# jonaselgammal/GPry

Measured on AMD Instinct MI355X. Metric: gp_refit_plus_nora_acq_cycle_throughput, higher is better.
Workload: dtype f64

## Files before the change

### gpry_amd/csrc/common.h

```cpp
#pragma once
#include <hip/hip_runtime.h>
#include <stdint.h>
#include <stdio.h>
#include <string.h>
#include <math.h>
#include <string>
#include <vector>
#include <map>

#include "../../include/gpry_hip.h"

#define GPRY_THETA_MAX (2 + GPRY_MAX_DIM)
#define GPRY_BPAR_ROW (2 + GPRY_MAX_DIM)
#define GPRY_BPAR_WHITE (1 + GPRY_MAX_DIM)
#define GPRY_TILE 128
#define GPRY_NB 64

typedef double v4d __attribute__((ext_vector_type(4)));

struct StageTimer {
    double total_ms = 0.0;
    int64_t count = 0;
    std::vector<std::pair<hipEvent_t, hipEvent_t>> pending;
};
// ... 65 lines not shown
    double* dalpha_ = nullptr;
    double* dvec = nullptr;
    int* dinfo = nullptr;
    double* dparams = nullptr;

    double* gate_sv = nullptr; double* gate_coef = nullptr; double* gate_trust = nullptr;
    int64_t gate_nsv = 0, gate_sv_cap = 0;
    double gate_gamma = 0.0, gate_intercept = 0.0;
    int gate_positive_finite = 1, gate_has_trust = 0, gates_on = 0;

    int64_t sw_M = 0, sw_cap = 0;
    double* dXc = nullptr;
    uint8_t* dmask = nullptr;
    double *dy_all = nullptr, *dsig_all = nullptr, *dacq_all = nullptr;
    struct CandSet {
        int64_t M = 0, cap = 0;
        double* dXc = nullptr; uint8_t* dmask = nullptr;
        double *dy = nullptr, *dsig = nullptr, *dacq = nullptr;
    } pr;
    double* dXcs = nullptr;
    int64_t xcs_cap = 0;
    double* dYcs = nullptr;
    int64_t ycs_cap = 0;
    double xcenter[GPRY_MAX_DIM] = {0};
    double xsum[GPRY_MAX_DIM] = {0};
    double xlo[GPRY_MAX_DIM] = {0}, xhi[GPRY_MAX_DIM] = {0};
    int opt_cross_mfma = 1;
    double alpha_l2 = -1.0;
    double alpha_l1 = 0.0;
    double noise_min = 0.0;
    int panel_form = 0;
    int opt_cross_hybrid = 1;
    double panel_est[4] = {0, 0, 0, 2.5e-7};
    double* dKst = nullptr;
    int64_t kst_cap = 0;
    double* dG = nullptr;
    int64_t g_cap = 0;
    double* dsplit = nullptr;
    int64_t split_cap = 0;
    int opt_predict_split = 1;
    int opt_gemm_dma = 1;
    double* dpart = nullptr;
    int64_t part_cap = 0;
    unsigned long long* dkeys = nullptr; int64_t keys_cap = 0;
    unsigned int* dhist = nullptr;
    unsigned int* dselp = nullptr;
// ... 26 lines not shown
    void* trtri_pipe = nullptr;
    int64_t opt_gemm_streamk = 5632;
    int64_t opt_topk_host = 16384;
    int opt_factor_pipeline = 1;
    int opt_factor_pipeline_min = 1280;
    void* chol_plan = nullptr;

    void* srv = nullptr;
    int opt_predict_serve = 1;
    int64_t opt_serve_idle_us = 2000;
    int opt_mcmc_mapped = 0;
    int64_t opt_chol_stacked = 2048;
    int opt_chol_stacked_dense = 0;
    int opt_sweep_overlap = 0;
    int opt_sweep_upload = 1;
    const double* up_X = nullptr;
    const double* up_y = nullptr;
    int up_gates = 0;
    int opt_kb_rank = 1;
    int opt_predict_gates = 0;
    int opt_sweep_prune = 0;
    int opt_sweep_mean_bound = 1;
    int opt_sweep_screen = 1;
    int sw_pruned = 0;
    struct PruneState {
        int have_mask = 0;
        int form = 0;
        FinishParams fp = {};
        int64_t n_eval = 0;
        int64_t rounds = 0, evaluated_total = 0, completed = 0, last_K = 0;
        int64_t n_gidx = 0;
        int tau_done = 0;
        double tau = 0.0;
        int64_t survivors = -1;
        int ybound = 0;
        int64_t live_blocks = 0, blocks = 0;
        int64_t cert_blocks = 0;
    } prune;
    struct ModelSnap {
        double *dV = nullptr, *dalpha_ = nullptr, *dXs = nullptr, *dX = nullptr;
        int64_t v_cap = 0, a_cap = 0, xs_cap = 0, x_cap = 0;
        int64_t N = 0, Np = 0;
        int d = 0, dpad = 0, kernel_id = 0;
        bool white = false;
        double theta[GPRY_THETA_MAX] = {0};
        gpry_affine tf;
// ... 159 lines not shown
void gemm_parts_plan_free(GemmPartsPlan* pl);
int gemm_dma_parts_launch(gpry_ctx* ctx, const GemmArgs& g, bool a_trans, bool b_trans, int epi, const GemmPartsPlan& pl,
                          int64_t slice_stride);
int gemm_f64_launch(gpry_ctx* ctx, const GemmArgs& g, bool a_trans, bool b_trans, int epi);
int gemm64_launch(gpry_ctx* ctx, const GemmArgs& g, bool a_trans, bool b_trans, int epi);
int gemm_split_scratch(gpry_ctx* ctx, int nsplit, int64_t slice, double** buf);
int launch_trtri_diag(gpry_ctx* ctx, const double* L, double* V, int64_t Np, hipStream_t st, bool zero_right = false);
int ensure_pred_xs(gpry_ctx* ctx);
int launch_point_full(gpry_ctx* ctx, const double* x, int want_kinv, double* kstar, double* G, double* u, double* part,
                      double* mean_part, double* ss_part, double* out);
int launch_trtri_diag128(gpry_ctx* ctx, const double* L, double* V, int64_t Np, hipStream_t st, bool clear_right);
int launch_trtri_diag_range(gpry_ctx* ctx, const double* L, double* V, int64_t Np, int blk0, int nblk, hipStream_t st);
bool gemm_dma_usable(const GemmArgs& g, int M, int N, int K);
int gemm_dma_launch_product(gpry_ctx* ctx, const GemmArgs& g, bool a_trans, bool b_trans, int epi, dim3 grid);
int sweep_gemm_dma_sp_launch(gpry_ctx* ctx, const GemmArgs& g);

int upload_params(gpry_ctx* ctx, const double* theta);
int launch_scale_train(gpry_ctx* ctx);
int launch_kernel_train(gpry_ctx* ctx, double* K, int add_noise, double* U = nullptr);
int launch_kernel_rows(gpry_ctx* ctx, int64_t row0, int k, int64_t ldk, double* Bk, double* Cb);
int launch_cross_build(gpry_ctx* ctx, const double* Xc, int64_t m0, int64_t mc,
                       int64_t ldk, double* Kst, double* mean_part, int raw_affine,
                       hipStream_t st = nullptr);
int launch_cross_prepare(gpry_ctx* ctx);
int launch_cross_build_mfma(gpry_ctx* ctx, const double* Xc, int64_t m0, int64_t mc, int64_t ldk, double* Kst, double* mean_part,
                            int raw_affine, int hybrid = 0);
int launch_cross_mean_bound(gpry_ctx* ctx, const double* Xc, int64_t m0, int64_t mc, double* mean_part, double* sabs_part,
                            double ubnd, double uhi, unsigned long long* live_cnt);
int launch_cross_build_small(gpry_ctx* ctx, const double* Xc, int64_t m0, int64_t mc, int64_t ldk,
                             double* Kst, double* mean_part, int raw_affine);
int launch_predict_mean_small(gpry_ctx* ctx, const double* Xc, int64_t M, int nsplit, double* part_out);
int launch_gates(gpry_ctx* ctx, const double* Xc, int64_t M, uint8_t* mask);
int launch_predict_small_std(gpry_ctx* ctx, const double* Xc, int M, double* kstar, double* mean_part,
                             double* ss_part);
int launch_gradx(gpry_ctx* ctx, const double* x, int raw_affine, int want_kinv, double* kstar, double* G,
                 double* u, double* w, double* part, double* out);
int launch_gradx_batch(gpry_ctx* ctx, const double* Xb, int64_t m, int raw_affine, const double* Wm, int64_t ldw,
                       double* out);
int launch_lml_small(gpry_ctx* ctx, int want_grad, double* out, int* info);
int launch_lml_small_batch(gpry_ctx* ctx, int B, const double* params, int want_grad, double* out, int* info);
int launch_lml_traces(gpry_ctx* ctx, const double* Kinv, const double* alpha,
                      double* grad_out_dev, const double* lq_dev, double* host_res, int info_at);

int potrf_lower_fused(gpry_ctx* ctx, double* A, int64_t Np);
int potrf_lower_overlap(gpry_ctx* ctx, double* A, int64_t Np);
int potrf_stacked(gpry_ctx* ctx, double* A, double* U, int64_t Np);
bool potrf_stacked_usable(const gpry_ctx* ctx, int64_t Np);
// ... 71 lines not shown
```

### gpry_amd/csrc/ctx.hip

```cpp
#include "common.h"
#include <string>
#include <stdarg.h>
#include <dlfcn.h>

thread_local char g_last_error[1024] = {0};
void trtri_plan_free(gpry_ctx* ctx);
void overlap_plan_free(gpry_ctx* ctx);

int gpry_fail(gpry_ctx* ctx, int code, const char* fmt, ...) {
    va_list ap;
    va_start(ap, fmt);
    vsnprintf(g_last_error, sizeof(g_last_error), fmt, ap);
    va_end(ap);
    if (ctx) { strncpy(ctx->err, g_last_error, sizeof(ctx->err) - 1); }
    return code;
}

template <typename T>
int dev_alloc(gpry_ctx* ctx, T** p, int64_t count) {
    *p = nullptr;
    if (count <= 0) count = 1;
    HIP_TRY(ctx, hipMalloc((void**)p, sizeof(T) * (size_t)count));
    return 0;
}
// ... 195 lines not shown
                return gpry_fail(nullptr, -1, "GPRY_HIP_OPTIONS: bad entry '%s'", item.c_str());
            }
        }
    }
    *out = ctx;
    return 0;
}

int gpry_ctx_destroy(gpry_ctx* ctx) {
    if (!ctx) return 0;
    (void)hipSetDevice(ctx->device);
    (void)hipStreamSynchronize(ctx->stream);
    if (ctx->stream2) (void)hipStreamSynchronize(ctx->stream2);
    timers_collect(ctx);
    serve_free(ctx);
    trtri_plan_free(ctx);
    trtri_pipe_free(ctx);
    overlap_plan_free(ctx);
    void* bufs[] = {ctx->dX, ctx->dXs, ctx->dy, ctx->dnoise, ctx->dA, ctx->dV, ctx->dW, ctx->dW2, ctx->dW3,
                    ctx->dalpha_, ctx->dvec, ctx->dinfo, ctx->dparams, ctx->dXc, ctx->dmask, ctx->dy_all,
                    ctx->dsig_all, ctx->dacq_all, ctx->dKst, ctx->dpart, ctx->dkeys, ctx->dhist, ctx->dselp,
                    ctx->dcand, ctx->dsel, ctx->dU, ctx->dXkb, ctx->dkbout, ctx->pr.dXc, ctx->pr.dmask,
                    ctx->pr.dy, ctx->pr.dsig, ctx->pr.dacq, ctx->dG,
                    ctx->gate_sv, ctx->gate_coef, ctx->gate_trust, ctx->dsplit, ctx->dbord, ctx->barena, ctx->dXcs, ctx->dYcs,
                    ctx->dub, ctx->dXg, ctx->dgidx, ctx->snap.dV, ctx->snap.dalpha_, ctx->snap.dXs, ctx->snap.dX, ctx->dmc, ctx->dknn,
                    ctx->dph, ctx->djoint, ctx->dloo, ctx->dsvm, ctx->dhess, ctx->dtg, ctx->dpw, ctx->dvtg};
    for (void* b : bufs) if (b) (void)hipFree(b);
    if (ctx->hpin) (void)hipHostFree(ctx->hpin);
    if (ctx->hloo) (void)hipHostFree(ctx->hloo);
    if (ctx->hsvm) (void)hipHostFree(ctx->hsvm);
    if (ctx->hbres) (void)hipHostFree(ctx->hbres);
    (void)hipStreamDestroy(ctx->stream);
    if (ctx->stream2) (void)hipStreamDestroy(ctx->stream2);
    for (hipEvent_t ev : ctx->ev_pool) (void)hipEventDestroy(ev);
    for (hipStream_t st : ctx->tp_streams) (void)hipStreamDestroy(st);
    for (hipEvent_t ev : ctx->tp_events) (void)hipEventDestroy(ev);
    delete ctx;
    return 0;
}

const char* gpry_last_error(gpry_ctx* ctx) { return ctx ? ctx->err : g_last_error; }

int gpry_ctx_sync(gpry_ctx* ctx) {
    if (!ctx) return gpry_fail(nullptr, -1, "gpry_ctx_sync: ctx is NULL");
    HIP_TRY(ctx, hipStreamSynchronize(ctx->stream));
    return 0;
}
// ... 20 lines not shown
    OPT_INT("gemm_small", opt_gemm_small, 0, BIG, c->lml_cache = false),
    OPT_INT("cross_mfma", opt_cross_mfma, 0, 1, (void)0),
    OPT_INT("cross_hybrid", opt_cross_hybrid, 0, 1, (void)0),
    OPT_INT("sweep_chunk", opt_sweep_chunk, 0, BIG, c->opt_sweep_chunk = round_up(c->opt_sweep_chunk, 1024)),
    OPT_INT("topk_host", opt_topk_host, 0, BIG, (void)0),
    OPT_INT("lml_small", opt_lml_small, 0, 1, c->lml_cache = false),
    OPT_INT("lml_cache", opt_lml_cache, 0, 1, c->lml_cache = false),
    OPT_INT("lml_batch", opt_lml_batch, 0, BIG, (void)0),
    OPT_INT("lml_batch_mb", opt_lml_batch_mb, 1, BIG, (void)0),
    OPT_INT("lml_schedule", opt_lml_schedule, 0, 1, (void)0),
    OPT_INT("lml_streams", opt_lml_streams, 1, 8, (void)0),
    OPT_INT("chol_tp_segments", opt_chol_tp_segments, 0, 1, c->lml_cache = false),
    OPT_INT("panel_debug", opt_panel_debug, 0, 511, c->lml_cache = false),
    OPT_INT("tp_left", opt_tp_left, 0, 1, (void)0),
    OPT_INT("tp_block", opt_tp_block, 128, BIG, c->opt_tp_block = round_up(c->opt_tp_block, 128); overlap_plan_free(c)),
    OPT_INT("tp_tail", opt_tp_tail, 128, BIG, c->opt_tp_tail = round_up(c->opt_tp_tail, 128); overlap_plan_free(c)),
    OPT_INT("predict_small", opt_predict_small, 0, BIG, (void)0),
    OPT_INT("predict_split", opt_predict_split, 0, 1, (void)0),
    OPT_INT("sweep_upload", opt_sweep_upload, 0, 1, (void)0),
    OPT_INT("sweep_overlap", opt_sweep_overlap, 0, 1, (void)0),
    OPT_INT("sweep_prune", opt_sweep_prune, 0, 1, (void)0),
    OPT_INT("sweep_mean_bound", opt_sweep_mean_bound, 0, 1, (void)0),
    OPT_INT("sweep_screen", opt_sweep_screen, 0, 1, (void)0),
    OPT_INT("sweep_small_map", opt_sweep_small_map, 0, 1, (void)0),
    OPT_INT("select_fused", opt_select_fused, 0, 1, (void)0),
    OPT_INT("prune_one_select", opt_prune_one_select, 0, 1, (void)0),
    OPT_INT("chol_stacked", opt_chol_stacked, 0, BIG, c->lml_cache = false),
    OPT_INT("chol_stacked_dense", opt_chol_stacked_dense, 0, 1, c->lml_cache = false),
    OPT_INT("predict_gates", opt_predict_gates, 0, 1, (void)0),
    OPT_INT("predict_serve", opt_predict_serve, 0, 1, (void)0),
    OPT_INT("serve_idle_us", opt_serve_idle_us, 10, 1000000, (void)0),
    OPT_INT("mcmc_mapped", opt_mcmc_mapped, 0, 1, (void)0),
    OPT_INT("kb_rank", opt_kb_rank, 0, 1, (void)0),
    OPT_INT("svm_iters_per_launch", opt_svm_iters, 1, BIG, (void)0),
};
#undef OPT_INT
const OptionSpec* find_option(const char* key) {
    for (const OptionSpec& o : OPTIONS) if (!strcmp(o.key, key)) return &o;
    return nullptr;
}
}

int gpry_ctx_set_option(gpry_ctx* ctx, const char* key, int64_t value) {
    if (!ctx || !key) return gpry_fail(ctx, -1, "gpry_ctx_set_option: NULL argument");
    GPRY_TRY(serve_stop(ctx));
    const OptionSpec* o = find_option(key);
// ... 376 lines not shown
```

### gpry_amd/csrc/kernel_build.hip

```cpp
#include "common.h"

#include "kern_math.h"

__global__ void scale_train_kernel(const double* __restrict__ X, double* __restrict__ Xs_,
                                   int64_t N, int64_t Np, int d, int dpad, AffParams ap, int* info_,
                                   const double* __restrict__ bpar, int64_t bstride) {
    const int tb = (int)blockIdx.z;
    double* __restrict__ Xs = bset(Xs_, tb, bstride);
    int* info = bset(info_, tb, bstride);
    int64_t idx = (int64_t)blockIdx.x * blockDim.x + threadIdx.x;
    if (idx < 4) info[idx] = 0;
    if (idx >= Np * dpad) return;
    int64_t i = idx / dpad; int k = (int)(idx - i * dpad);
    double v = 0.0;
    if (i < N && k < d) v = X[i * d + k] / (bpar ? bset(bpar, tb, bstride)[1 + k] : ap.ls[k]);
    Xs[idx] = v;
}

int launch_scale_train(gpry_ctx* ctx) {
    AffParams ap = make_ap(ctx, false);
    int64_t n = ctx->Np * ctx->dpad;
    hipLaunchKernelGGL(scale_train_kernel, dim3((unsigned)((n + 255) / 256), 1, (unsigned)ctx->bn), dim3(256), 0,
                       ctx->stream, ctx->dX, ctx->dXs, ctx->N, ctx->Np, ctx->d, ctx->dpad, ap, ctx->dinfo, ctx->bpar, ctx->bstride);
    HIP_TRY(ctx, hipGetLastError());
// ... 218 lines not shown
        if (in_chunk && Kst) {
#pragma unroll
            for (int q = 0; q < 4; q++) Kst[((int64_t)jc * 128 + j0 + q) * ldk + ml] = v[q];
        }
    }
    for (int jj = nfull; jj < 128; jj++) {
        double v = 0.0;
        if (jj < nvalid) {
            double r2 = 0.0;
#pragma unroll
            for (int k = 0; k < DP; k++) {
                double df = xs[k] - Xl[jj * DP + k];
                r2 = fma(df, df, r2);
            }
            v = kp.C * corr_r2_fast<KID>(r2);
            macc = fma(al[jj], v, macc);
        }
        if (in_chunk && Kst) Kst[((int64_t)jc * 128 + jj) * ldk + ml] = v;
    }
    if (in_chunk && mean_part) mean_part[(int64_t)jc * mc + ml] = macc;
}

template <int DP, int KID, bool HYB, bool BND = false>
__global__ __launch_bounds__(256) void cross_build_mfma_kernel(
    const double* __restrict__ Xcs, int64_t ldm, int64_t mc,
    const double* __restrict__ Ycs, const double* __restrict__ alpha_,
    double* __restrict__ Kst, int64_t ldk, double* __restrict__ mean_part, KernParams kp, double ucut,
    double ubnd = 0.0, double uhi = 0.0, double* __restrict__ sabs_part = nullptr,
    unsigned long long* __restrict__ live_cnt = nullptr, int screen = 0) {
    typedef float v4f __attribute__((ext_vector_type(4)));
    constexpr int S = DP + 2, KS = DP / 4;
    constexpr double SC = corr_scale<KID>();
    __shared__ __attribute__((aligned(16))) double Yl[128 * S];
    __shared__ double yn[128], al[128];
    constexpr int SF = DP + 1;
    __shared__ float Yf[BND ? 128 * SF : 1];
    const int t = threadIdx.x, lane = t & 63, w = t >> 6, r = lane & 15, g = lane >> 4;
    const int jc = blockIdx.y;
    const int64_t mb = (int64_t)blockIdx.x * 256 + 64 * w;
    for (int e = t; e < 128 * (DP / 2); e += 256) {
        const int row = e / (DP / 2), k2 = (e - row * (DP / 2)) * 2;
        const double2 v = *reinterpret_cast<const double2*>(Ycs + ((int64_t)jc * 128 + row) * DP + k2);
        *reinterpret_cast<double2*>(Yl + row * S + k2) = v;
        if (BND) { Yf[row * SF + k2] = (float)v.x; Yf[row * SF + k2 + 1] = (float)v.y; }
    }
    if (t < 128) al[t] = alpha_ ? alpha_[jc * 128 + t] : 0.0;
    double xb[4][KS], xn[4];
    float xbf[4][KS];
#pragma unroll
    for (int tp = 0; tp < 2; tp++) {
        double s0 = 0.0, s1 = 0.0;
#pragma unroll
        for (int kk = 0; kk < KS; kk++) {
            const double2 v = *reinterpret_cast<const double2*>(Xcs + (int64_t)(4 * kk + g) * ldm + mb + 32 * tp + 2 * r);
            xb[2 * tp][kk] = v.x; xb[2 * tp + 1][kk] = v.y;
            if (BND) { xbf[2 * tp][kk] = (float)v.x; xbf[2 * tp + 1][kk] = (float)v.y; }
            s0 = fma(v.x, v.x, s0); s1 = fma(v.y, v.y, s1);
        }
        s0 += __shfl_xor(s0, 16); s0 += __shfl_xor(s0, 32);
        s1 += __shfl_xor(s1, 16); s1 += __shfl_xor(s1, 32);
        xn[2 * tp] = s0 * SC; xn[2 * tp + 1] = s1 * SC;
    }
    __syncthreads();
    if (t < 128) {
        double s = 0.0;
#pragma unroll
        for (int k = 0; k < DP; k++) s = fma(Yl[t * S + k], Yl[t * S + k], s);
        yn[t] = s * SC;
    }
    __syncthreads();
    const int64_t left = kp.N - (int64_t)jc * 128;
    const int nvalid = left >= 128 ? 128 : (left > 0 ? (int)left : 0);
    double macc[4] = {0.0, 0.0, 0.0, 0.0};
    double sacc[4] = {0.0, 0.0, 0.0, 0.0};
    unsigned nlive = 0, nfall = 0;
    bool scr = false;
    float lo32 = 0.0f, hi32 = 0.0f;
    if (BND && screen) {
        const double y0 = yn[lane], y1 = yn[lane + 64];
        bool bad = !(y0 <= 1e36) || !(y1 <= 1e36);
        double ym = fmax(y0, y1), xm = fmax(fmax(xn[0], xn[1]), fmax(xn[2], xn[3]));
#pragma unroll
        for (int tl = 0; tl < 4; tl++) bad = bad || !(xn[tl] <= 1e36);
#pragma unroll
        for (int o = 1; o < 64; o <<= 1) { ym = fmax(ym, __shfl_xor(ym, o)); xm = fmax(xm, __shfl_xor(xm, o)); }
        const double rs = sqrt(ym) + sqrt(xm);
        const double delta = 5.9604644775390625e-08 * (double)(kp.d + 8) * rs * rs;
        const double lo = ubnd + delta, hi = uhi - delta;
        lo32 = (float)lo;
        if ((double)lo32 < lo) lo32 = __uint_as_float(__float_as_uint(lo32) + 1u);
        hi32 = (float)hi;
        if ((double)hi32 > hi) hi32 = __uint_as_float(__float_as_uint(hi32) - 1u);
        scr = !__any(bad || !(hi > 0.0) || !(lo32 <= hi32));
        lo32 = __uint_as_float(__builtin_amdgcn_readfirstlane(__float_as_uint(lo32)));
        hi32 = __uint_as_float(__builtin_amdgcn_readfirstlane(__float_as_uint(hi32)));
    }
#pragma unroll 1
    for (int j0 = 0; j0 < 128; j0 += 16) {
        double a[KS], ynq[4], alq[4];
        if (!BND) {
#pragma unroll
            for (int kk = 0; kk < KS; kk++) a[kk] = Yl[(j0 + r) * S + 4 * kk + g];
#pragma unroll
            for (int q = 0; q < 4; q++) { ynq[q] = yn[j0 + g + 4 * q]; alq[q] = al[j0 + g + 4 * q]; }
        }
#pragma unroll
        for (int tp = 0; tp < 2; tp++) {
            if (BND && scr) {
                float af[KS];
                double yns[4];
#pragma unroll
                for (int kk = 0; kk < KS; kk++) af[kk] = Yf[(j0 + r) * SF + 4 * kk + g];
#pragma unroll
                for (int i = 0; i < 4; i++) yns[i] = yn[j0 + 4 * g + i];
                v4f c0 = {0.0f, 0.0f, 0.0f, 0.0f}, c1 = {0.0f, 0.0f, 0.0f, 0.0f};
#pragma unroll
                for (int kk = 0; kk < KS; kk++) {
                    c0 = __builtin_amdgcn_mfma_f32_16x16x4f32(af[kk], xbf[2 * tp][kk], c0, 0, 0, 0);
                    c1 = __builtin_amdgcn_mfma_f32_16x16x4f32(af[kk], xbf[2 * tp + 1][kk], c1, 0, 0, 0);
                }
                float mn = __builtin_inff(), mx = -__builtin_inff();
#pragma unroll
                for (int i = 0; i < 4; i++) {
                    const float w0 = fmaf(-2.0f * (float)SC, c0[i], (float)(xn[2 * tp] + yns[i]));
                    const float w1 = fmaf(-2.0f * (float)SC, c1[i], (float)(xn[2 * tp + 1] + yns[i]));
                    mn = fminf(mn, fminf(w0, w1)); mx = fmaxf(mx, fmaxf(w0, w1));
                }
                if (!__any(!(mn >= lo32 && mx <= hi32))) continue;
            }
            if (BND) {
#pragma unroll
                for (int kk = 0; kk < KS; kk++) a[kk] = Yl[(j0 + r) * S + 4 * kk + g];
#pragma unroll
                for (int q = 0; q < 4; q++) { ynq[q] = yn[j0 + g + 4 * q]; alq[q] = al[j0 + g + 4 * q]; }
            }
            v4d acc0 = {0.0, 0.0, 0.0, 0.0}, acc1 = {0.0, 0.0, 0.0, 0.0};
#pragma unroll
            for (int kk = 0; kk < KS; kk++) acc0 = __builtin_amdgcn_mfma_f64_16x16x4f64(a[kk], xb[2 * tp][kk], acc0, 0, 0, 0);
#pragma unroll
            for (int kk = 0; kk < KS; kk++) acc1 = __builtin_amdgcn_mfma_f64_16x16x4f64(a[kk], xb[2 * tp + 1][kk], acc1, 0, 0, 0);
            const int64_t mloc = mb + 32 * tp + 2 * r;
            const bool in_chunk = mloc < mc;
            double ue0[4], ue1[4];
            bool live = false;
#pragma unroll
            for (int q = 0; q < 4; q++) {
                ue0[q] = fma(-2.0 * SC, acc0[q], xn[2 * tp] + ynq[q]);
                ue1[q] = fma(-2.0 * SC, acc1[q], xn[2 * tp + 1] + ynq[q]);
                if (BND) live = live || !(ue0[q] >= ubnd && ue0[q] <= uhi) || !(ue1[q] >= ubnd && ue1[q] <= uhi);
            }
            if (BND) {
                if (!__any(live)) { if (screen) nfall++; continue; }
                nlive++;
            }
#pragma unroll
            for (int q = 0; q < 4; q++) {
                const int jj = j0 + g + 4 * q;
                double u0 = ue0[q];
                double u1 = ue1[q];
                if (HYB && (u0 < ucut || u1 < ucut)) {
                    double r0 = 0.0, r1 = 0.0;
#pragma unroll 2
                    for (int k = 0; k < DP; k++) {
                        const double yk = Yl[jj * S + k];
                        const double2 xk = *reinterpret_cast<const double2*>(Xcs + (int64_t)k * ldm + mloc);
                        const double d0 = xk.x - yk, d1 = xk.y - yk;
                        r0 = fma(d0, d0, r0); r1 = fma(d1, d1, r1);
                    }
                    u0 = r0 * SC; u1 = r1 * SC;
                }
                u0 = fmax(u0, 1e-290);
                u1 = fmax(u1, 1e-290);
                double v0 = kp.C * corr_scaled_fast<KID>(u0);
                double v1 = kp.C * corr_scaled_fast<KID>(u1);
                if (jj >= nvalid) { v0 = 0.0; v1 = 0.0; }
                macc[2 * tp] = fma(alq[q], v0, macc[2 * tp]);
                macc[2 * tp + 1] = fma(alq[q], v1, macc[2 * tp + 1]);
                if (BND) {
                    sacc[2 * tp] = fma(fabs(alq[q]), fabs(v0), sacc[2 * tp]);
                    sacc[2 * tp + 1] = fma(fabs(alq[q]), fabs(v1), sacc[2 * tp + 1]);
                }
                if (in_chunk && Kst) *reinterpret_cast<double2*>(Kst + ((int64_t)jc * 128 + jj) * ldk + mloc) = make_double2(v0, v1);
            }
        }
    }
    if (mean_part) {
#pragma unroll
        for (int tl = 0; tl < 4; tl++) {
            double s = macc[tl];
            s += __shfl_xor(s, 16);
            s += __shfl_xor(s, 32);
            const int64_t ml = mb + 32 * (tl >> 1) + 2 * r + (tl & 1);
            if (g == 0 && ml < mc) mean_part[(int64_t)jc * mc + ml] = s;
            if (BND) {
                double sa = sacc[tl];
                sa += __shfl_xor(sa, 16);
                sa += __shfl_xor(sa, 32);
                if (g == 0 && ml < mc) sabs_part[(int64_t)jc * mc + ml] = sa;
            }
        }
    }
    if (BND && lane == 0 && nlive) atomicAdd(live_cnt, (unsigned long long)nlive);
    if (BND && lane == 0 && nfall) atomicAdd(live_cnt + 1, (unsigned long long)nfall);
}
__global__ __launch_bounds__(256) void center_train_kernel(const double* __restrict__ X, double* __restrict__ Ycs, int64_t N, int64_t Np, int d,
                                                           int dsel, AffParams ap, AffParams cen) {
    const int64_t idx = (int64_t)blockIdx.x * blockDim.x + threadIdx.x;
    if (idx >= Np * dsel) return;
    const int64_t i = idx / dsel;
    const int k = (int)(idx - i * dsel);
    Ycs[idx] = (i < N && k < d) ? (X[i * d + k] - cen.lo[k]) / ap.ls[k] : 0.0;
}
__global__ __launch_bounds__(256) void center_cand_kernel(const double* __restrict__ Xc, int64_t M, int64_t m0, int64_t mc, int d, int dsel,
                                                          int has_aff, AffParams ap, AffParams cen, double* __restrict__ Xcs, int64_t ldm) {
    const int64_t idx = (int64_t)blockIdx.x * blockDim.x + threadIdx.x;
    if (idx >= mc * dsel) return;
    const int64_t ml = idx / dsel;
    const int k = (int)(idx - ml * dsel);
    const int64_t m = m0 + ml;
    double v = 0.0;
    if (k < d && m < M) {
        v = Xc[m * d + k];
        if (has_aff) v = (v - ap.lo[k]) / ap.span[k];
        v = (v - cen.lo[k]) / ap.ls[k];
    }
    Xcs[(int64_t)k * ldm + ml] = v;
}

int launch_cross_prepare(gpry_ctx* ctx) {
    const int dsel = dp_class(ctx->d);
    if (ctx->Np * dsel > ctx->ycs_cap) {
        if (ctx->dYcs) GPRY_TRY(dev_free(ctx, ctx->dYcs));
        ctx->dYcs = nullptr; ctx->ycs_cap = 0;
        GPRY_TRY(dev_alloc(ctx, &ctx->dYcs, ctx->Np * dsel));
        ctx->ycs_cap = ctx->Np * dsel;
    }
    AffParams ap = make_ap(ctx, false), cen;
    for (int k = 0; k < GPRY_MAX_DIM; k++) { cen.ls[k] = 1.0; cen.span[k] = 1.0; cen.lo[k] = k < ctx->d ? ctx->xcenter[k] : 0.0; }
    hipLaunchKernelGGL(center_train_kernel, dim3((unsigned)((ctx->Np * dsel + 255) / 256)), dim3(256), 0, ctx->stream, ctx->dX, ctx->dYcs,
                       ctx->N, ctx->Np, ctx->d, dsel, ap, cen);
    HIP_TRY(ctx, hipGetLastError());
    return 0;
}

static int center_cands(gpry_ctx* ctx, const double* Xc, int64_t m0, int64_t mc, int raw_affine, KernParams* kp, int* dsel_,
                        int64_t* ldm_) {
    *kp = make_kp(ctx);
    kp->has_aff = raw_affine && ctx->tf.has_x_affine;
    AffParams ap = make_ap(ctx, kp->has_aff), cen;
    for (int k = 0; k < GPRY_MAX_DIM; k++) { cen.ls[k] = 1.0; cen.span[k] = 1.0; cen.lo[k] = k < ctx->d ? ctx->xcenter[k] : 0.0; }
    if (ctx->d > 32) return gpry_fail(ctx, -1, "d > 32 is not supported");
    const int dsel = dp_class(ctx->d);
    const int64_t ldm = round_up(mc, 256);
    if (dsel * ldm > ctx->xcs_cap) {
        if (ctx->dXcs) GPRY_TRY(dev_free(ctx, ctx->dXcs));
        ctx->dXcs = nullptr; ctx->xcs_cap = 0;
        GPRY_TRY(dev_alloc(ctx, &ctx->dXcs, dsel * ldm));
        ctx->xcs_cap = dsel * ldm;
    }
    hipLaunchKernelGGL(center_cand_kernel, dim3((unsigned)((ldm * dsel + 255) / 256)), dim3(256), 0, ctx->stream, Xc, ctx->sw_M, m0, ldm,
                       ctx->d, dsel, kp->has_aff, ap, cen, ctx->dXcs, ldm);
    *dsel_ = dsel; *ldm_ = ldm;
    return 0;
}
// ... 8 lines not shown
    dim3 grid((unsigned)((mc + 255) / 256), (unsigned)(ctx->Np / 128));
#define CM2(DP, KID) do { const double ucut = 100.0 * corr_scale<KID>();                                                                  \
                       if (hybrid) { hipLaunchKernelGGL((cross_build_mfma_kernel<DP, KID, true>), grid, dim3(256), 0, st, ctx->dXcs, ldm, mc, ctx->dYcs, \
                                                        ctx->dalpha_, Kst, ldk, mean_part, kp, ucut); }                                  \
                       else { hipLaunchKernelGGL((cross_build_mfma_kernel<DP, KID, false>), grid, dim3(256), 0, st, ctx->dXcs, ldm, mc, ctx->dYcs, \
                                                 ctx->dalpha_, Kst, ldk, mean_part, kp, ucut); } } while (0)
#define CM4(KID) { if (dsel == 4) CM2(4, KID); else if (dsel == 8) CM2(8, KID); else if (dsel == 16) CM2(16, KID); \
                   else if (dsel == 24) CM2(24, KID); else CM2(32, KID); }
    DISPATCH_KID(ctx->kernel_id, CM4)
#undef CM4
#undef CM2
    HIP_TRY(ctx, hipGetLastError());
    return 0;
}

int launch_cross_mean_bound(gpry_ctx* ctx, const double* Xc, int64_t m0, int64_t mc, double* mean_part, double* sabs_part,
                            double ubnd, double uhi, unsigned long long* live_cnt) {
    const int screen = ctx->opt_sweep_screen;
    hipStream_t st = ctx->stream;
    KernParams kp;
    int dsel = 0;
    int64_t ldm = 0;
    GPRY_TRY(center_cands(ctx, Xc, m0, mc, 1, &kp, &dsel, &ldm));
    dim3 grid((unsigned)((mc + 255) / 256), (unsigned)(ctx->Np / 128));
#define CB2(DP, KID) hipLaunchKernelGGL((cross_build_mfma_kernel<DP, KID, true, true>), grid, dim3(256), 0, st, ctx->dXcs, ldm, mc, ctx->dYcs, \
                                        ctx->dalpha_, nullptr, mc, mean_part, kp, 100.0 * corr_scale<KID>(), ubnd, uhi, sabs_part, live_cnt, screen)
#define CB4(KID) { if (dsel == 4) CB2(4, KID); else if (dsel == 8) CB2(8, KID); else if (dsel == 16) CB2(16, KID); \
                   else if (dsel == 24) CB2(24, KID); else CB2(32, KID); }
    DISPATCH_KID(ctx->kernel_id, CB4)
#undef CB4
#undef CB2
    HIP_TRY(ctx, hipGetLastError());
    return 0;
}

template <int DP, int KID>
__global__ __launch_bounds__(256) void cross_build_small_kernel(
    const double* __restrict__ Xc, int64_t M, int64_t m0, int64_t mc,
    const double* __restrict__ Xs, const double* __restrict__ alpha_,
    double* __restrict__ Kst, int64_t ldk, double* __restrict__ mean_part,
    KernParams kp, AffParams ap) {
    __shared__ double Xl[128 * DP];
    __shared__ double al[128];
    const int t = threadIdx.x, rg = t >> 6;
    const int64_t ml = (int64_t)blockIdx.x * 64 + (t & 63);
    const int64_t m = m0 + ml;
    const int jc = blockIdx.y;
    for (int e = t; e < 128 * DP; e += 256) {
        int row = e / DP, k = e - row * DP;
// ... 786 lines not shown
```

### gpry_amd/csrc/sweep.hip

```cpp
#include "sweep.h"
#include "acq_math.h"
#include <algorithm>

__global__ void logexp_kernel(const double* __restrict__ mu, const double* __restrict__ sd, int64_t n, double zeta,
                              double baseline, double sigma_n, double* __restrict__ acq) {
    int64_t i = (int64_t)blockIdx.x * blockDim.x + threadIdx.x;
    if (i < n) acq[i] = logexp_value(mu[i], sd[i], zeta, baseline, sigma_n);
}
int launch_logexp(gpry_ctx* ctx, const double* mu, const double* sd, int64_t n, double zeta, double baseline, double sigma_n, double* acq) {
    hipLaunchKernelGGL(logexp_kernel, dim3((unsigned)((n + 255) / 256)), dim3(256), 0, ctx->stream, mu, sd, n, zeta, baseline, sigma_n, acq);
    HIP_TRY(ctx, hipGetLastError());
    return 0;
}

__device__ __forceinline__ double sum_partials(const double* __restrict__ part, int nt, int64_t ldp, int64_t col) {
    double s = 0.0;
#pragma unroll 8
    for (int t = 0; t < nt; t++) s += part[(int64_t)t * ldp + col];
    return s;
}
__device__ __forceinline__ double finish_y(double mu_, unsigned mk, const FinishParams& fp) {
    double y = mu_ * fp.y_std + fp.y_mean;
    y = fmin(y, fp.clip_hi);
    if (mk) y = -INFINITY;
// ... 281 lines not shown
    fp.clip_hi = ctx->tf.clip_hi; fp.zeta = rq.zeta; fp.baseline = rq.baseline; fp.sigma_n = rq.sigma_n;
    fp.want_std = rq.kind != SWEEP_PREDICT || rq.want_std; fp.want_acq = rq.kind != SWEEP_PREDICT;
    return fp;
}

int run_sweep(gpry_ctx* ctx, int64_t M, const SweepRequest& rq) {
    const bool predict = rq.kind == SWEEP_PREDICT, stage_a = rq.kind == SWEEP_STAGE_A, y_given = rq.y_given;
    const int64_t Np = ctx->Np;
    const int nt = (int)(Np / 128);
    const int64_t chunk = sweep_chunk(ctx, M);
    const bool overlap = ctx->opt_sweep_overlap && ctx->stream2 != nullptr && rq.kind == SWEEP_FULL && M > chunk;
    const int nbuf = overlap ? 2 : 1;
    if (stage_a) GPRY_TRY(dev_grow(ctx, &ctx->dub, &ctx->ub_cap, round_up(M, 1024)));
    else GPRY_TRY(dev_grow(ctx, &ctx->dKst, &ctx->kst_cap, nbuf * Np * chunk));
    const bool small_build = predict && M <= 512;
    const int nt_mean = small_build ? 4 * nt : nt;
    const int64_t part_stride = (int64_t)(nt_mean + nt) * chunk;
    GPRY_TRY(ensure_part(ctx, nbuf * part_stride));
    const FinishParams fp = finish_params(ctx, rq);
    ctx->sw_M = M;
    GPRY_TRY(choose_panel_form(ctx, small_build));
    const int form = ctx->panel_form;
    const bool no_panel = stage_a && y_given;
    if (panel_from_matrix_pipe(form) && !no_panel) GPRY_TRY(launch_cross_prepare(ctx));
    if (stage_a) ctx->prune.form = form;
    const MeanBound mb = mean_bound_setup(ctx, rq, fp, nt);
    unsigned long long* live_cnt = nullptr;
    if (stage_a) { ctx->prune.ybound = mb.on ? 1 : 0; ctx->prune.live_blocks = 0; ctx->prune.blocks = 0; ctx->prune.cert_blocks = 0; }
    if (mb.on) {
        if (!ctx->dsel) GPRY_TRY(dev_alloc(ctx, &ctx->dsel, gpry_ctx::DSEL_WORDS));
        live_cnt = ctx->dsel + gpry_ctx::DSEL_LIVE;
        HIP_TRY(ctx, hipMemsetAsync(live_cnt, 0, 16, ctx->stream));
        if (getenv("GPRY_HIP_DEBUG_PANEL"))
            fprintf(stderr, "gpry: bound pass: u in [%.6g, %.3g] skipped, D %.3g, gamma %.3g\n", mb.ubnd, mb.uhi, mb.D1, mb.g3 / 3.0);
    }
    const double* up_X = ctx->up_X;
    const double* up_y = ctx->up_y;
    const size_t nchunk = (size_t)((M + chunk - 1) / chunk);
    if (up_X || overlap) {
        while (ctx->ev_pool.size() < 3 * nchunk + 1) {
            hipEvent_t ev;
            HIP_TRY(ctx, hipEventCreateWithFlags(&ev, hipEventDisableTiming));
            ctx->ev_pool.push_back(ev);
        }
    }
    const hipStream_t main_stream = ctx->stream, side = ctx->stream2;
    struct StreamSwap {
        gpry_ctx* c; hipStream_t keep;
        StreamSwap(gpry_ctx* ctx, hipStream_t st) : c(ctx), keep(ctx->stream) { c->stream = st; }
// ... 336 lines not shown
```

Baseline: 66.75 million.

## Walk several training tiles per block in bound pass with precomputed train operands

Adds a prepass kernel that computes the training-side squared norms, per-tile max norm and bad flags, and a float32 copy of the centered training points once per prepare. The bound-pass cross-build kernel then reads these instead of recomputing them per block. Each block walks several consecutive training tiles (default two), reusing its candidate registers. The f32 screening now uses four MFMA accumulators so both halves are screened together. It also sets occupancy launch bounds on the bound variant. The cost is fewer blocks in the grid, an extra small kernel and buffer, and more register pressure.

```diff
diff --git a/gpry_amd/csrc/common.h b/gpry_amd/csrc/common.h
--- a/gpry_amd/csrc/common.h
+++ b/gpry_amd/csrc/common.h
@@ -111,6 +111,8 @@
     int64_t xcs_cap = 0;
     double* dYcs = nullptr;
     int64_t ycs_cap = 0;
+    double* dYop = nullptr;
+    int64_t yop_cap = 0;
     double xcenter[GPRY_MAX_DIM] = {0};
     double xsum[GPRY_MAX_DIM] = {0};
     double xlo[GPRY_MAX_DIM] = {0}, xhi[GPRY_MAX_DIM] = {0};
@@ -183,6 +185,7 @@
     int opt_sweep_prune = 0;
     int opt_sweep_mean_bound = 1;
     int opt_sweep_screen = 1;
+    int opt_sweep_bound_walk = 2;
     int sw_pruned = 0;
     struct PruneState {
         int have_mask = 0;
@@ -388,7 +391,7 @@
 int launch_cross_build(gpry_ctx* ctx, const double* Xc, int64_t m0, int64_t mc,
                        int64_t ldk, double* Kst, double* mean_part, int raw_affine,
                        hipStream_t st = nullptr);
-int launch_cross_prepare(gpry_ctx* ctx);
+int launch_cross_prepare(gpry_ctx* ctx, bool bound_ops = false);
 int launch_cross_build_mfma(gpry_ctx* ctx, const double* Xc, int64_t m0, int64_t mc, int64_t ldk, double* Kst, double* mean_part,
                             int raw_affine, int hybrid = 0);
 int launch_cross_mean_bound(gpry_ctx* ctx, const double* Xc, int64_t m0, int64_t mc, double* mean_part, double* sabs_part,
diff --git a/gpry_amd/csrc/ctx.hip b/gpry_amd/csrc/ctx.hip
--- a/gpry_amd/csrc/ctx.hip
+++ b/gpry_amd/csrc/ctx.hip
@@ -241,7 +241,7 @@
                     ctx->dsig_all, ctx->dacq_all, ctx->dKst, ctx->dpart, ctx->dkeys, ctx->dhist, ctx->dselp,
                     ctx->dcand, ctx->dsel, ctx->dU, ctx->dXkb, ctx->dkbout, ctx->pr.dXc, ctx->pr.dmask,
                     ctx->pr.dy, ctx->pr.dsig, ctx->pr.dacq, ctx->dG,
-                    ctx->gate_sv, ctx->gate_coef, ctx->gate_trust, ctx->dsplit, ctx->dbord, ctx->barena, ctx->dXcs, ctx->dYcs,
+                    ctx->gate_sv, ctx->gate_coef, ctx->gate_trust, ctx->dsplit, ctx->dbord, ctx->barena, ctx->dXcs, ctx->dYcs, ctx->dYop,
                     ctx->dub, ctx->dXg, ctx->dgidx, ctx->snap.dV, ctx->snap.dalpha_, ctx->snap.dXs, ctx->snap.dX, ctx->dmc, ctx->dknn,
                     ctx->dph, ctx->djoint, ctx->dloo, ctx->dsvm, ctx->dhess, ctx->dtg, ctx->dpw, ctx->dvtg};
     for (void* b : bufs) if (b) (void)hipFree(b);
@@ -308,6 +308,7 @@
     OPT_INT("sweep_prune", opt_sweep_prune, 0, 1, (void)0),
     OPT_INT("sweep_mean_bound", opt_sweep_mean_bound, 0, 1, (void)0),
     OPT_INT("sweep_screen", opt_sweep_screen, 0, 1, (void)0),
+    OPT_INT("sweep_bound_walk", opt_sweep_bound_walk, 1, 64, (void)0),
     OPT_INT("sweep_small_map", opt_sweep_small_map, 0, 1, (void)0),
     OPT_INT("select_fused", opt_select_fused, 0, 1, (void)0),
     OPT_INT("prune_one_select", opt_prune_one_select, 0, 1, (void)0),
diff --git a/gpry_amd/csrc/kernel_build.hip b/gpry_amd/csrc/kernel_build.hip
--- a/gpry_amd/csrc/kernel_build.hip
+++ b/gpry_amd/csrc/kernel_build.hip
@@ -264,12 +264,14 @@
 }
 
 template <int DP, int KID, bool HYB, bool BND = false>
-__global__ __launch_bounds__(256) void cross_build_mfma_kernel(
+__global__ __launch_bounds__(256, BND ? (DP == 4 ? 4 : DP <= 16 ? 3 : 2) : 0) void cross_build_mfma_kernel(
     const double* __restrict__ Xcs, int64_t ldm, int64_t mc,
     const double* __restrict__ Ycs, const double* __restrict__ alpha_,
     double* __restrict__ Kst, int64_t ldk, double* __restrict__ mean_part, KernParams kp, double ucut,
     double ubnd = 0.0, double uhi = 0.0, double* __restrict__ sabs_part = nullptr,
-    unsigned long long* __restrict__ live_cnt = nullptr, int screen = 0) {
+    unsigned long long* __restrict__ live_cnt = nullptr, int screen = 0,
+    const float* __restrict__ Yf32 = nullptr, const double* __restrict__ ynp = nullptr, const double* __restrict__ ych = nullptr,
+    int walk = 1, int nt = 0) {
     typedef float v4f __attribute__((ext_vector_type(4)));
     constexpr int S = DP + 2, KS = DP / 4;
     constexpr double SC = corr_scale<KID>();
@@ -278,15 +280,22 @@
     constexpr int SF = DP + 1;
     __shared__ float Yf[BND ? 128 * SF : 1];
     const int t = threadIdx.x, lane = t & 63, w = t >> 6, r = lane & 15, g = lane >> 4;
-    const int jc = blockIdx.y;
+    int jc = BND ? blockIdx.y * walk : blockIdx.y;
+    const int jc1 = BND ? (jc + walk < nt ? jc + walk : nt) : 0;
     const int64_t mb = (int64_t)blockIdx.x * 256 + 64 * w;
-    for (int e = t; e < 128 * (DP / 2); e += 256) {
-        const int row = e / (DP / 2), k2 = (e - row * (DP / 2)) * 2;
-        const double2 v = *reinterpret_cast<const double2*>(Ycs + ((int64_t)jc * 128 + row) * DP + k2);
-        *reinterpret_cast<double2*>(Yl + row * S + k2) = v;
-        if (BND) { Yf[row * SF + k2] = (float)v.x; Yf[row * SF + k2 + 1] = (float)v.y; }
-    }
-    if (t < 128) al[t] = alpha_ ? alpha_[jc * 128 + t] : 0.0;
+#define CROSS_FILL(JC)                                                                                                        \
+    for (int e = t; e < 128 * (DP / 2); e += 256) {                                                                           \
+        const int row = e / (DP / 2), k2 = (e - row * (DP / 2)) * 2;                                                          \
+        const double2 v = *reinterpret_cast<const double2*>(Ycs + ((int64_t)(JC) * 128 + row) * DP + k2);                     \
+        *reinterpret_cast<double2*>(Yl + row * S + k2) = v;                                                                   \
+        if (BND) {                                                                                                            \
+            const float2 f = *reinterpret_cast<const float2*>(Yf32 + ((int64_t)(JC) * 128 + row) * DP + k2);                  \
+            Yf[row * SF + k2] = f.x; Yf[row * SF + k2 + 1] = f.y;                                                             \
+        }                                                                                                                     \
+    }                                                                                                                         \
+    if (t < 128) al[t] = alpha_ ? alpha_[(JC) * 128 + t] : 0.0;                                                               \
+    if (BND && t < 128) yn[t] = ynp[(JC) * 128 + t];
+    CROSS_FILL(jc)
     double xb[4][KS], xn[4];
     float xbf[4][KS];
 #pragma unroll
@@ -303,51 +312,58 @@
         s1 += __shfl_xor(s1, 16); s1 += __shfl_xor(s1, 32);
         xn[2 * tp] = s0 * SC; xn[2 * tp + 1] = s1 * SC;
     }
-    __syncthreads();
-    if (t < 128) {
-        double s = 0.0;
-#pragma unroll
-        for (int k = 0; k < DP; k++) s = fma(Yl[t * S + k], Yl[t * S + k], s);
-        yn[t] = s * SC;
-    }
-    __syncthreads();
-    const int64_t left = kp.N - (int64_t)jc * 128;
-    const int nvalid = left >= 128 ? 128 : (left > 0 ? (int)left : 0);
-    double macc[4] = {0.0, 0.0, 0.0, 0.0};
-    double sacc[4] = {0.0, 0.0, 0.0, 0.0};
+    double sxm = 0.0;
+    bool badx = false;
+    if (BND && screen) {
+        double xm = fmax(fmax(xn[0], xn[1]), fmax(xn[2], xn[3]));
+#pragma unroll
+        for (int tl = 0; tl < 4; tl++) badx = badx || !(xn[tl] <= 1e36);
+#pragma unroll
+        for (int o = 1; o < 64; o <<= 1) xm = fmax(xm, __shfl_xor(xm, o));
+        sxm = sqrt(xm);
+    }
     unsigned nlive = 0, nfall = 0;
-    bool scr = false;
-    float lo32 = 0.0f, hi32 = 0.0f;
-    if (BND && screen) {
-        const double y0 = yn[lane], y1 = yn[lane + 64];
-        bool bad = !(y0 <= 1e36) || !(y1 <= 1e36);
-        double ym = fmax(y0, y1), xm = fmax(fmax(xn[0], xn[1]), fmax(xn[2], xn[3]));
-#pragma unroll
-        for (int tl = 0; tl < 4; tl++) bad = bad || !(xn[tl] <= 1e36);
-#pragma unroll
-        for (int o = 1; o < 64; o <<= 1) { ym = fmax(ym, __shfl_xor(ym, o)); xm = fmax(xm, __shfl_xor(xm, o)); }
-        const double rs = sqrt(ym) + sqrt(xm);
-        const double delta = 5.9604644775390625e-08 * (double)(kp.d + 8) * rs * rs;
-        const double lo = ubnd + delta, hi = uhi - delta;
-        lo32 = (float)lo;
-        if ((double)lo32 < lo) lo32 = __uint_as_float(__float_as_uint(lo32) + 1u);
-        hi32 = (float)hi;
-        if ((double)hi32 > hi) hi32 = __uint_as_float(__float_as_uint(hi32) - 1u);
-        scr = !__any(bad || !(hi > 0.0) || !(lo32 <= hi32));
-        lo32 = __uint_as_float(__builtin_amdgcn_readfirstlane(__float_as_uint(lo32)));
-        hi32 = __uint_as_float(__builtin_amdgcn_readfirstlane(__float_as_uint(hi32)));
-    }
+    do {
+        __syncthreads();
+        if (!BND) {
+            if (t < 128) {
+                double s = 0.0;
+#pragma unroll
+                for (int k = 0; k < DP; k++) s = fma(Yl[t * S + k], Yl[t * S + k], s);
+                yn[t] = s * SC;
+            }
+            __syncthreads();
+        }
+        const int64_t left = kp.N - (int64_t)jc * 128;
+        const int nvalid = left >= 128 ? 128 : (left > 0 ? (int)left : 0);
+        double macc[4] = {0.0, 0.0, 0.0, 0.0};
+        double sacc[4] = {0.0, 0.0, 0.0, 0.0};
+        bool scr = false;
+        float lo32 = 0.0f, hi32 = 0.0f;
+        if (BND && screen) {
+            const double ym = ych[2 * jc];
+            const bool bad = badx || ych[2 * jc + 1] != 0.0;
+            const double rs = sqrt(ym) + sxm;
+            const double delta = 5.9604644775390625e-08 * (double)(kp.d + 8) * rs * rs;
+            const double lo = ubnd + delta, hi = uhi - delta;
+            lo32 = (float)lo;
+            if ((double)lo32 < lo) lo32 = __uint_as_float(__float_as_uint(lo32) + 1u);
+            hi32 = (float)hi;
+            if ((double)hi32 > hi) hi32 = __uint_as_float(__float_as_uint(hi32) - 1u);
+            scr = !__any(bad || !(hi > 0.0) || !(lo32 <= hi32));
+            lo32 = __uint_as_float(__builtin_amdgcn_readfirstlane(__float_as_uint(lo32)));
+            hi32 = __uint_as_float(__builtin_amdgcn_readfirstlane(__float_as_uint(hi32)));
+        }
 #pragma unroll 1
-    for (int j0 = 0; j0 < 128; j0 += 16) {
-        double a[KS], ynq[4], alq[4];
-        if (!BND) {
-#pragma unroll
-            for (int kk = 0; kk < KS; kk++) a[kk] = Yl[(j0 + r) * S + 4 * kk + g];
-#pragma unroll
-            for (int q = 0; q < 4; q++) { ynq[q] = yn[j0 + g + 4 * q]; alq[q] = al[j0 + g + 4 * q]; }
-        }
-#pragma unroll
-        for (int tp = 0; tp < 2; tp++) {
+        for (int j0 = 0; j0 < 128; j0 += 16) {
+            double a[KS], ynq[4], alq[4];
+            if (!BND) {
+#pragma unroll
+                for (int kk = 0; kk < KS; kk++) a[kk] = Yl[(j0 + r) * S + 4 * kk + g];
+#pragma unroll
+                for (int q = 0; q < 4; q++) { ynq[q] = yn[j0 + g + 4 * q]; alq[q] = al[j0 + g + 4 * q]; }
+            }
+            bool cert[2] = {false, false};
             if (BND && scr) {
                 float af[KS];
                 double yns[4];
@@ -355,93 +371,107 @@
                 for (int kk = 0; kk < KS; kk++) af[kk] = Yf[(j0 + r) * SF + 4 * kk + g];
 #pragma unroll
                 for (int i = 0; i < 4; i++) yns[i] = yn[j0 + 4 * g + i];
-                v4f c0 = {0.0f, 0.0f, 0.0f, 0.0f}, c1 = {0.0f, 0.0f, 0.0f, 0.0f};
+                v4f c[4];
+#pragma unroll
+                for (int tl = 0; tl < 4; tl++) c[tl] = v4f{0.0f, 0.0f, 0.0f, 0.0f};
 #pragma unroll
                 for (int kk = 0; kk < KS; kk++) {
-                    c0 = __builtin_amdgcn_mfma_f32_16x16x4f32(af[kk], xbf[2 * tp][kk], c0, 0, 0, 0);
-                    c1 = __builtin_amdgcn_mfma_f32_16x16x4f32(af[kk], xbf[2 * tp + 1][kk], c1, 0, 0, 0);
+#pragma unroll
+                    for (int tl = 0; tl < 4; tl++) c[tl] = __builtin_amdgcn_mfma_f32_16x16x4f32(af[kk], xbf[tl][kk], c[tl], 0, 0, 0);
                 }
-                float mn = __builtin_inff(), mx = -__builtin_inff();
-#pragma unroll
-                for (int i = 0; i < 4; i++) {
-                    const float w0 = fmaf(-2.0f * (float)SC, c0[i], (float)(xn[2 * tp] + yns[i]));
-                    const float w1 = fmaf(-2.0f * (float)SC, c1[i], (float)(xn[2 * tp + 1] + yns[i]));
-                    mn = fminf(mn, fminf(w0, w1)); mx = fmaxf(mx, fmaxf(w0, w1));
+#pragma unroll
+                for (int tp = 0; tp < 2; tp++) {
+                    float mn = __builtin_inff(), mx = -__builtin_inff();
+#pragma unroll
+                    for (int i = 0; i < 4; i++) {
+                        const float w0 = fmaf(-2.0f * (float)SC, c[2 * tp][i], (float)(xn[2 * tp] + yns[i]));
+                        const float w1 = fmaf(-2.0f * (float)SC, c[2 * tp + 1][i], (float)(xn[2 * tp + 1] + yns[i]));
+                        mn = fminf(mn, fminf(w0, w1)); mx = fmaxf(mx, fmaxf(w0, w1));
+                    }
+                    cert[tp] = !__any(!(mn >= lo32 && mx <= hi32));
                 }
-                if (!__any(!(mn >= lo32 && mx <= hi32))) continue;
-            }
-            if (BND) {
-#pragma unroll
-                for (int kk = 0; kk < KS; kk++) a[kk] = Yl[(j0 + r) * S + 4 * kk + g];
-#pragma unroll
-                for (int q = 0; q < 4; q++) { ynq[q] = yn[j0 + g + 4 * q]; alq[q] = al[j0 + g + 4 * q]; }
-            }
-            v4d acc0 = {0.0, 0.0, 0.0, 0.0}, acc1 = {0.0, 0.0, 0.0, 0.0};
-#pragma unroll
-            for (int kk = 0; kk < KS; kk++) acc0 = __builtin_amdgcn_mfma_f64_16x16x4f64(a[kk], xb[2 * tp][kk], acc0, 0, 0, 0);
-#pragma unroll
-            for (int kk = 0; kk < KS; kk++) acc1 = __builtin_amdgcn_mfma_f64_16x16x4f64(a[kk], xb[2 * tp + 1][kk], acc1, 0, 0, 0);
-            const int64_t mloc = mb + 32 * tp + 2 * r;
-            const bool in_chunk = mloc < mc;
-            double ue0[4], ue1[4];
-            bool live = false;
-#pragma unroll
-            for (int q = 0; q < 4; q++) {
-                ue0[q] = fma(-2.0 * SC, acc0[q], xn[2 * tp] + ynq[q]);
-                ue1[q] = fma(-2.0 * SC, acc1[q], xn[2 * tp + 1] + ynq[q]);
-                if (BND) live = live || !(ue0[q] >= ubnd && ue0[q] <= uhi) || !(ue1[q] >= ubnd && ue1[q] <= uhi);
-            }
-            if (BND) {
-                if (!__any(live)) { if (screen) nfall++; continue; }
-                nlive++;
-            }
-#pragma unroll
-            for (int q = 0; q < 4; q++) {
-                const int jj = j0 + g + 4 * q;
-                double u0 = ue0[q];
-                double u1 = ue1[q];
-                if (HYB && (u0 < ucut || u1 < ucut)) {
-                    double r0 = 0.0, r1 = 0.0;
+            }
+#pragma unroll
+            for (int tp = 0; tp < 2; tp++) {
+                if (BND && cert[tp]) continue;
+                if (BND) {
+#pragma unroll
+                    for (int kk = 0; kk < KS; kk++) a[kk] = Yl[(j0 + r) * S + 4 * kk + g];
+#pragma unroll
+                    for (int q = 0; q < 4; q++) { ynq[q] = yn[j0 + g + 4 * q]; alq[q] = al[j0 + g + 4 * q]; }
+                }
+                v4d acc0 = {0.0, 0.0, 0.0, 0.0}, acc1 = {0.0, 0.0, 0.0, 0.0};
+#pragma unroll
+                for (int kk = 0; kk < KS; kk++) acc0 = __builtin_amdgcn_mfma_f64_16x16x4f64(a[kk], xb[2 * tp][kk], acc0, 0, 0, 0);
+#pragma unroll
+                for (int kk = 0; kk < KS; kk++) acc1 = __builtin_amdgcn_mfma_f64_16x16x4f64(a[kk], xb[2 * tp + 1][kk], acc1, 0, 0, 0);
+                const int64_t mloc = mb + 32 * tp + 2 * r;
+                const bool in_chunk = mloc < mc;
+                double ue0[4], ue1[4];
+                bool live = false;
+#pragma unroll
+                for (int q = 0; q < 4; q++) {
+                    ue0[q] = fma(-2.0 * SC, acc0[q], xn[2 * tp] + ynq[q]);
+                    ue1[q] = fma(-2.0 * SC, acc1[q], xn[2 * tp + 1] + ynq[q]);
+                    if (BND) live = live || !(ue0[q] >= ubnd && ue0[q] <= uhi) || !(ue1[q] >= ubnd && ue1[q] <= uhi);
+                }
+                if (BND) {
+                    if (!__any(live)) { if (screen) nfall++; continue; }
+                    nlive++;
+                }
+#pragma unroll
+                for (int q = 0; q < 4; q++) {
+                    const int jj = j0 + g + 4 * q;
+                    double u0 = ue0[q];
+                    double u1 = ue1[q];
+                    if (HYB && (u0 < ucut || u1 < ucut)) {
+                        double r0 = 0.0, r1 = 0.0;
 #pragma unroll 2
-                    for (int k = 0; k < DP; k++) {
-                        const double yk = Yl[jj * S + k];
-                        const double2 xk = *reinterpret_cast<const double2*>(Xcs + (int64_t)k * ldm + mloc);
-                        const double d0 = xk.x - yk, d1 = xk.y - yk;
-                        r0 = fma(d0, d0, r0); r1 = fma(d1, d1, r1);
+                        for (int k = 0; k < DP; k++) {
+                            const double yk = Yl[jj * S + k];
+                            const double2 xk = *reinterpret_cast<const double2*>(Xcs + (int64_t)k * ldm + mloc);
+                            const double d0 = xk.x - yk, d1 = xk.y - yk;
+                            r0 = fma(d0, d0, r0); r1 = fma(d1, d1, r1);
+                        }
+                        u0 = r0 * SC; u1 = r1 * SC;
                     }
-                    u0 = r0 * SC; u1 = r1 * SC;
+                    u0 = fmax(u0, 1e-290);
+                    u1 = fmax(u1, 1e-290);
+                    double v0 = kp.C * corr_scaled_fast<KID>(u0);
+                    double v1 = kp.C * corr_scaled_fast<KID>(u1);
+                    if (jj >= nvalid) { v0 = 0.0; v1 = 0.0; }
+                    macc[2 * tp] = fma(alq[q], v0, macc[2 * tp]);
+                    macc[2 * tp + 1] = fma(alq[q], v1, macc[2 * tp + 1]);
+                    if (BND) {
+                        sacc[2 * tp] = fma(fabs(alq[q]), fabs(v0), sacc[2 * tp]);
+                        sacc[2 * tp + 1] = fma(fabs(alq[q]), fabs(v1), sacc[2 * tp + 1]);
+                    }
+                    if (in_chunk && Kst) *reinterpret_cast<double2*>(Kst + ((int64_t)jc * 128 + jj) * ldk + mloc) = make_double2(v0, v1);
                 }
-                u0 = fmax(u0, 1e-290);
-                u1 = fmax(u1, 1e-290);
-                double v0 = kp.C * corr_scaled_fast<KID>(u0);
-                double v1 = kp.C * corr_scaled_fast<KID>(u1);
-                if (jj >= nvalid) { v0 = 0.0; v1 = 0.0; }
-                macc[2 * tp] = fma(alq[q], v0, macc[2 * tp]);
-                macc[2 * tp + 1] = fma(alq[q], v1, macc[2 * tp + 1]);
+            }
+        }
+        if (mean_part) {
+#pragma unroll
+            for (int tl = 0; tl < 4; tl++) {
+                double s = macc[tl];
+                s += __shfl_xor(s, 16);
+                s += __shfl_xor(s, 32);
+                const int64_t ml = mb + 32 * (tl >> 1) + 2 * r + (tl & 1);
+                if (g == 0 && ml < mc) mean_part[(int64_t)jc * mc + ml] = s;
                 if (BND) {
-                    sacc[2 * tp] = fma(fabs(alq[q]), fabs(v0), sacc[2 * tp]);
-                    sacc[2 * tp + 1] = fma(fabs(alq[q]), fabs(v1), sacc[2 * tp + 1]);
+                    double sa = sacc[tl];
+                    sa += __shfl_xor(sa, 16);
+                    sa += __shfl_xor(sa, 32);
+                    if (g == 0 && ml < mc) sabs_part[(int64_t)jc * mc + ml] = sa;
                 }
-                if (in_chunk && Kst) *reinterpret_cast<double2*>(Kst + ((int64_t)jc * 128 + jj) * ldk + mloc) = make_double2(v0, v1);
-            }
-        }
-    }
-    if (mean_part) {
-#pragma unroll
-        for (int tl = 0; tl < 4; tl++) {
-            double s = macc[tl];
-            s += __shfl_xor(s, 16);
-            s += __shfl_xor(s, 32);
-            const int64_t ml = mb + 32 * (tl >> 1) + 2 * r + (tl & 1);
-            if (g == 0 && ml < mc) mean_part[(int64_t)jc * mc + ml] = s;
-            if (BND) {
-                double sa = sacc[tl];
-                sa += __shfl_xor(sa, 16);
-                sa += __shfl_xor(sa, 32);
-                if (g == 0 && ml < mc) sabs_part[(int64_t)jc * mc + ml] = sa;
-            }
-        }
-    }
+            }
+        }
+        if (BND && jc + 1 < jc1) {
+            __syncthreads();
+            CROSS_FILL(jc + 1)
+        }
+    } while (BND && ++jc < jc1);
+#undef CROSS_FILL
     if (BND && lane == 0 && nlive) atomicAdd(live_cnt, (unsigned long long)nlive);
     if (BND && lane == 0 && nfall) atomicAdd(live_cnt + 1, (unsigned long long)nfall);
 }
@@ -452,6 +482,27 @@
     const int64_t i = idx / dsel;
     const int k = (int)(idx - i * dsel);
     Ycs[idx] = (i < N && k < d) ? (X[i * d + k] - cen.lo[k]) / ap.ls[k] : 0.0;
+}
+__global__ __launch_bounds__(128) void train_bound_ops_kernel(const double* __restrict__ Ycs, int dsel, double sc, double* __restrict__ yn,
+                                                              double* __restrict__ ych, float* __restrict__ Yf) {
+    __shared__ double wmax[2];
+    __shared__ int wbad[2];
+    const int t = threadIdx.x, jc = blockIdx.x;
+    const int64_t i = (int64_t)jc * 128 + t;
+    double s = 0.0;
+    for (int k = 0; k < dsel; k++) {
+        const double v = Ycs[i * dsel + k];
+        Yf[i * dsel + k] = (float)v;
+        s = fma(v, v, s);
+    }
+    const double n = __dmul_rn(s, sc);
+    yn[i] = n;
+    double m = n;
+    const bool bad = __any(!(n <= 1e36)) != 0;
+    for (int o = 1; o < 64; o <<= 1) m = fmax(m, __shfl_xor(m, o));
+    if ((t & 63) == 0) { wmax[t >> 6] = m; wbad[t >> 6] = bad ? 1 : 0; }
+    __syncthreads();
+    if (t == 0) { ych[2 * jc] = fmax(wmax[0], wmax[1]); ych[2 * jc + 1] = (wbad[0] | wbad[1]) ? 1.0 : 0.0; }
 }
 __global__ __launch_bounds__(256) void center_cand_kernel(const double* __restrict__ Xc, int64_t M, int64_t m0, int64_t mc, int d, int dsel,
                                                           int has_aff, AffParams ap, AffParams cen, double* __restrict__ Xcs, int64_t ldm) {
@@ -469,7 +520,11 @@
     Xcs[(int64_t)k * ldm + ml] = v;
 }
 
-int launch_cross_prepare(gpry_ctx* ctx) {
+static double* bound_ops_yn(const gpry_ctx* ctx) { return ctx->dYop; }
+static double* bound_ops_ych(const gpry_ctx* ctx) { return ctx->dYop + ctx->Np; }
+static float* bound_ops_yf(const gpry_ctx* ctx) { return reinterpret_cast<float*>(ctx->dYop + ctx->Np + 2 * (ctx->Np / 128)); }
+
+int launch_cross_prepare(gpry_ctx* ctx, bool bound_ops) {
     const int dsel = dp_class(ctx->d);
     if (ctx->Np * dsel > ctx->ycs_cap) {
         if (ctx->dYcs) GPRY_TRY(dev_free(ctx, ctx->dYcs));
@@ -482,6 +537,17 @@
     hipLaunchKernelGGL(center_train_kernel, dim3((unsigned)((ctx->Np * dsel + 255) / 256)), dim3(256), 0, ctx->stream, ctx->dX, ctx->dYcs,
                        ctx->N, ctx->Np, ctx->d, dsel, ap, cen);
     HIP_TRY(ctx, hipGetLastError());
+    if (bound_ops) {
+        const int64_t nt = ctx->Np / 128;
+        GPRY_TRY(dev_grow(ctx, &ctx->dYop, &ctx->yop_cap, ctx->Np + 2 * nt + (ctx->Np * dsel + 1) / 2));
+        double sc = 0.0;
+#define SCK(KID) sc = corr_scale<KID>();
+        DISPATCH_KID(ctx->kernel_id, SCK)
+#undef SCK
+        hipLaunchKernelGGL(train_bound_ops_kernel, dim3((unsigned)nt), dim3(128), 0, ctx->stream, ctx->dYcs, dsel, sc, bound_ops_yn(ctx),
+                           bound_ops_ych(ctx), bound_ops_yf(ctx));
+        HIP_TRY(ctx, hipGetLastError());
+    }
     return 0;
 }
 
@@ -536,9 +602,13 @@
     int dsel = 0;
     int64_t ldm = 0;
     GPRY_TRY(center_cands(ctx, Xc, m0, mc, 1, &kp, &dsel, &ldm));
-    dim3 grid((unsigned)((mc + 255) / 256), (unsigned)(ctx->Np / 128));
+    const int nt = (int)(ctx->Np / 128), walk = ctx->opt_sweep_bound_walk < 1 ? 1 : ctx->opt_sweep_bound_walk;
+    if (!ctx->dYop || ctx->yop_cap < ctx->Np + 2 * nt + (ctx->Np * dsel + 1) / 2)
+        return gpry_fail(ctx, -1, "bound pass: the training-side operands were not prepared");
+    dim3 grid((unsigned)((mc + 255) / 256), (unsigned)((nt + walk - 1) / walk));
 #define CB2(DP, KID) hipLaunchKernelGGL((cross_build_mfma_kernel<DP, KID, true, true>), grid, dim3(256), 0, st, ctx->dXcs, ldm, mc, ctx->dYcs, \
-                                        ctx->dalpha_, nullptr, mc, mean_part, kp, 100.0 * corr_scale<KID>(), ubnd, uhi, sabs_part, live_cnt, screen)
+                                        ctx->dalpha_, nullptr, mc, mean_part, kp, 100.0 * corr_scale<KID>(), ubnd, uhi, sabs_part, live_cnt, screen, \
+                                        bound_ops_yf(ctx), bound_ops_yn(ctx), bound_ops_ych(ctx), walk, nt)
 #define CB4(KID) { if (dsel == 4) CB2(4, KID); else if (dsel == 8) CB2(8, KID); else if (dsel == 16) CB2(16, KID); \
                    else if (dsel == 24) CB2(24, KID); else CB2(32, KID); }
     DISPATCH_KID(ctx->kernel_id, CB4)
diff --git a/gpry_amd/csrc/sweep.hip b/gpry_amd/csrc/sweep.hip
--- a/gpry_amd/csrc/sweep.hip
+++ b/gpry_amd/csrc/sweep.hip
@@ -327,9 +327,9 @@
     GPRY_TRY(choose_panel_form(ctx, small_build));
     const int form = ctx->panel_form;
     const bool no_panel = stage_a && y_given;
-    if (panel_from_matrix_pipe(form) && !no_panel) GPRY_TRY(launch_cross_prepare(ctx));
     if (stage_a) ctx->prune.form = form;
     const MeanBound mb = mean_bound_setup(ctx, rq, fp, nt);
+    if (panel_from_matrix_pipe(form) && !no_panel) GPRY_TRY(launch_cross_prepare(ctx, mb.on));
     unsigned long long* live_cnt = nullptr;
     if (stage_a) { ctx->prune.ybound = mb.on ? 1 : 0; ctx->prune.live_blocks = 0; ctx->prune.blocks = 0; ctx->prune.cert_blocks = 0; }
     if (mb.on) {
```

After: 70.02 million, median of 4. 1.05x the previous value.
